# QuentinFuxa/WhisperLiveKit

Hardware: AMD Instinct MI355X
Metric: audio seconds transcribed per second (1/RTF), Whisper-base EN simul_whisper AlignAtt, 0.5 s chunks (higher is better)
Workload: dtype f32; 1 GPU; base.en simul_whisper, 1 stream(s) over 1 GPU(s) (1 per GPU), 30 s 16 kHz speech-like stream, 0.5 s chunks, beam 1, frame_threshold 25, seeded random weights, synthetic vocabulary; model=base.en, streams_total=1

## Files before the change

### include/wlk_hip.h

```cpp
#ifndef WLK_HIP_H
#define WLK_HIP_H

#include <stdint.h>

#ifdef __cplusplus
extern "C" {
#endif

#define WLK_OK 0
#define WLK_ERR_ARG (-1)
#define WLK_ERR_HIP (-2)
#define WLK_ERR_STATE (-3)
#define WLK_ERR_CAPACITY (-4)

typedef struct wlk_model wlk_model;
typedef struct wlk_session wlk_session;

typedef struct wlk_dims {
    int32_t n_mels, n_audio_ctx, n_audio_state, n_audio_head, n_audio_layer;
    int32_t n_vocab, n_text_ctx, n_text_state, n_text_head, n_text_layer;
} wlk_dims;

const char* wlk_last_error(void);
int wlk_abi_version(void);
int wlk_device_count(void);

int wlk_arena_floats(const wlk_dims* dims, uint64_t* n_floats);
int wlk_tensor_lookup(const wlk_dims* dims, const char* packed_name, uint64_t* offset_floats,
                      uint64_t* numel);
int wlk_tensor_name(const wlk_dims* dims, int index, const char** name);

int wlk_model_create(const wlk_dims* dims, int device, float* arena_dev, wlk_model** out);
int wlk_model_arena(wlk_model* m, float** arena_dev, uint64_t* n_floats);
int wlk_model_upload(wlk_model* m, const char* packed_name, const float* host, uint64_t numel);
int wlk_model_set_alignment_heads(wlk_model* m, const int32_t* layer_head_pairs, int n_pairs);
int wlk_model_finalize(wlk_model* m);
int wlk_model_destroy(wlk_model* m);

int wlk_session_create(wlk_model* m, int beam, int max_audio_samples, wlk_session** out);
int wlk_session_destroy(wlk_session* s);
// ... 180 lines not shown
int wlk_diag_linear_time(int m, int n, int k, int flags, int force_gemv, int reps, float* us_per_launch);
int wlk_diag_linear_ln(const float* a, const float* w, const float* bias, const float* gamma, const float* beta,
                       int m, int n, int k, int force_gemv, float* c);
int wlk_diag_layernorm(const float* x, const float* gamma, const float* beta, int rows, int d, float* y);
int wlk_diag_prefill_stack(wlk_session** sessions, const int64_t* tokens, const int32_t* n_tok, const int32_t* sot_index, int32_t n,
                           int32_t* taken);
int wlk_engine_prefill_stats(wlk_model* m, uint64_t* batches, uint64_t* sessions);
int wlk_diag_encoder_attention_time(int t, int d, int n_head, int k_splits, int reps, float* us_per_launch);
int wlk_diag_encoder_attention(const float* qkv, int t, int d, int n_head, float* out);
int wlk_diag_wave_ops(const float* in64, float* out640, float* ref640);
int wlk_diag_linear_x3(const float* a, const float* w, const float* bias, int m, int n, int k, int flags, float scale,
                       int scale_cols, float* c);
int wlk_diag_linear_x3_time(int m, int n, int k, int flags, int reps, float* us_per_launch);
int wlk_diag_layernorm_x3(const float* x, const float* gamma, const float* beta, int rows, int d, float* y);
int wlk_diag_encoder_attention_x3(const float* qkv, int t, int d, int n_head, float* out);
int wlk_diag_encoder_attention_x3_time(int t, int d, int n_head, int reps, float* us_per_launch);
int wlk_diag_qkv_x3_attention(const float* x, const float* w, const float* bias, int t, int d, int n_head, float scale,
                              float* out_epilogue, float* out_packed);

#ifdef __cplusplus
}
#endif
#endif
```

### whisperlivekit_amd/_lib.py

```python
from __future__ import annotations

import ctypes as C
import os
import threading
from typing import Optional


_LIB_NAME = "libwlk_hip.so"
_lock = threading.Lock()
_lib: Optional[C.CDLL] = None


class WlkError(RuntimeError):
    """Raised for every non-zero status of the C ABI (message from wlk_last_error())."""


class Dims(C.Structure):
    _fields_ = [(n, C.c_int32) for n in (
        "n_mels", "n_audio_ctx", "n_audio_state", "n_audio_head", "n_audio_layer",
        "n_vocab", "n_text_ctx", "n_text_state", "n_text_head", "n_text_layer")]


class SfDims(C.Structure):
    _fields_ = [(n, C.c_int32) for n in (
# ... 45 lines not shown
    os.environ["GPU_MAX_HW_QUEUES"] = str(int(n))
    return True


def lib_path() -> str:
    return os.environ.get("WLK_HIP_LIB", os.path.join(os.path.dirname(os.path.abspath(__file__)), _LIB_NAME))


def _declare(lib: C.CDLL) -> None:
    p, i32, u64, f32p, i32p = C.c_void_p, C.c_int32, C.c_uint64, C.POINTER(C.c_float), C.POINTER(C.c_int32)
    cint = C.c_int
    sig = {
        "wlk_last_error": (C.c_char_p, []),
        "wlk_abi_version": (cint, []),
        "wlk_device_count": (cint, []),
        "wlk_arena_floats": (cint, [C.POINTER(Dims), C.POINTER(u64)]),
        "wlk_tensor_lookup": (cint, [C.POINTER(Dims), C.c_char_p, C.POINTER(u64), C.POINTER(u64)]),
        "wlk_tensor_name": (cint, [C.POINTER(Dims), cint, C.POINTER(C.c_char_p)]),
        "wlk_model_create": (cint, [C.POINTER(Dims), cint, p, C.POINTER(p)]),
        "wlk_model_arena": (cint, [p, C.POINTER(p), C.POINTER(u64)]),
        "wlk_model_upload": (cint, [p, C.c_char_p, p, u64]),
        "wlk_model_set_alignment_heads": (cint, [p, p, cint]),
        "wlk_model_finalize": (cint, [p]),
        "wlk_model_destroy": (cint, [p]),
        "wlk_session_create": (cint, [p, cint, cint, C.POINTER(p)]),
        "wlk_session_destroy": (cint, [p]),
        "wlk_session_set_debug": (cint, [p, cint]),
        "wlk_audio_append": (cint, [p, p, cint]),
        "wlk_audio_append_pcm16": (cint, [p, p, cint]),
        "wlk_audio_append_zeros": (cint, [p, cint]),
# ... 75 lines not shown
        "wlk_log_mel": (cint, [C.c_void_p, C.POINTER(C.c_float), C.c_int64, C.c_int32, C.POINTER(C.c_float), C.c_uint64,
                               C.POINTER(C.c_int32)]),
        "wlk_find_alignment": (cint, [C.c_void_p, C.POINTER(C.c_int64), C.c_int32, C.c_int32, C.c_int32, C.c_int32, C.c_float,
                                      C.POINTER(C.c_float), C.POINTER(C.c_int8), C.POINTER(C.c_float)]),
        "wlk_diag_linear_time": (cint, [cint, cint, cint, cint, cint, cint, C.POINTER(C.c_float)]),
        "wlk_diag_linear_ln": (cint, [p, p, p, p, p, cint, cint, cint, cint, p]),
        "wlk_diag_layernorm": (cint, [p, p, p, cint, cint, p]),
        "wlk_diag_encoder_attention_time": (cint, [cint, cint, cint, cint, cint, C.POINTER(C.c_float)]),
        "wlk_diag_encoder_attention": (cint, [p, cint, cint, cint, p]),
        "wlk_diag_wave_ops": (cint, [p, p, p]),
        "wlk_diag_env_refresh": (cint, []),
        "wlk_diag_linear_x3": (cint, [p, p, p, cint, cint, cint, cint, C.c_float, cint, p]),
        "wlk_diag_linear_x3_time": (cint, [cint, cint, cint, cint, cint, C.POINTER(C.c_float)]),
        "wlk_diag_layernorm_x3": (cint, [p, p, p, cint, cint, p]),
        "wlk_diag_encoder_attention_x3": (cint, [p, cint, cint, cint, p]),
        "wlk_diag_encoder_attention_x3_time": (cint, [cint, cint, cint, cint, C.POINTER(C.c_float)]),
        "wlk_diag_qkv_x3_attention": (cint, [p, p, p, cint, cint, cint, C.c_float, p, p]),
    }
    for name, (res, args) in sig.items():
        try:
            fn = getattr(lib, name)
        except AttributeError:
            if "WLK_HIP_LIB" in os.environ and name.startswith("wlk_diag_"):
                continue
            raise
        fn.restype = res
        fn.argtypes = args


EXPORTED_SYMBOLS = (
    "wlk_last_error", "wlk_abi_version", "wlk_device_count", "wlk_arena_floats", "wlk_tensor_lookup",
    "wlk_tensor_name", "wlk_model_create", "wlk_model_arena", "wlk_model_upload",
    "wlk_model_set_alignment_heads", "wlk_model_finalize", "wlk_model_destroy", "wlk_session_create",
    "wlk_session_destroy", "wlk_session_set_debug", "wlk_audio_append", "wlk_audio_append_pcm16", "wlk_audio_append_zeros",
    "wlk_audio_drop_front", "wlk_audio_clear", "wlk_audio_len", "wlk_encode", "wlk_decode",
    "wlk_no_speech_prob", "wlk_rules_set", "wlk_pick_greedy", "wlk_select", "wlk_kv_reorder", "wlk_sync", "wlk_decode_until_stop", "wlk_engine_attach", "wlk_engine_detach",
    "wlk_engine_stats", "wlk_engine_encode_stats", "wlk_engine_prefill_stats", "wlk_diag_prefill_stack", "wlk_job_create",
    "wlk_job_begin_step", "wlk_job_no_speech", "wlk_job_adjustments", "wlk_job_consume", "wlk_job_result",
    "wlk_job_destroy", "wlk_export", "wlk_session_step_stats", "wlk_prof_begin",
    "wlk_prof_end", "wlk_melspec_create", "wlk_melspec_run", "wlk_melspec_destroy",
    "wlk_sf_arena_floats", "wlk_sf_tensor_lookup", "wlk_sf_tensor_name", "wlk_sf_create", "wlk_sf_upload",
    "wlk_sf_finalize", "wlk_sf_step", "wlk_sf_step_pcm", "wlk_sf_stats", "wlk_sf_export", "wlk_sf_destroy",
    "wlk_vad_weights_floats", "wlk_vad_tensor_lookup", "wlk_vad_tensor_name", "wlk_vad_create", "wlk_vad_destroy",
    "wlk_vad_stream_create", "wlk_vad_stream_reset", "wlk_vad_stream_run", "wlk_vad_stream_state",
    "wlk_vad_stream_destroy",
    "wlk_dtw", "wlk_encode_mel", "wlk_log_mel", "wlk_find_alignment",
    "wlk_nllb_arena_floats", "wlk_nllb_tensor_lookup", "wlk_nllb_tensor_name", "wlk_nllb_create", "wlk_nllb_upload",
    "wlk_nllb_finalize", "wlk_nllb_destroy", "wlk_nllb_session_create", "wlk_nllb_session_destroy", "wlk_nllb_encode",
    "wlk_nllb_decode", "wlk_nllb_step", "wlk_nllb_kv_reorder", "wlk_nllb_topk", "wlk_nllb_export", "wlk_nllb_sync",
    "wlk_diag_last_error", "wlk_diag_linear", "wlk_diag_linear_time", "wlk_diag_linear_ln", "wlk_diag_layernorm",
    "wlk_diag_encoder_attention", "wlk_diag_encoder_attention_time", "wlk_diag_wave_ops", "wlk_diag_env_refresh",
    "wlk_diag_linear_x3", "wlk_diag_linear_x3_time", "wlk_diag_layernorm_x3",
    "wlk_diag_encoder_attention_x3", "wlk_diag_encoder_attention_x3_time", "wlk_diag_qkv_x3_attention",
)


def load() -> C.CDLL:
    global _lib
    if _lib is not None:
        return _lib
    with _lock:
        if _lib is None:
            path = lib_path()
            if not os.path.exists(path):
                raise WlkError(
                    f"{path} not found: build it with `python -m whisperlivekit_amd.build` "
                    "(hipcc, gfx950). There is no CPU fallback for the HIP backend.")
            try:
# ... 21 lines not shown
```

### whisperlivekit_amd/csrc/api.hip

```cpp
#include <cmath>
#include <cstdio>
#include <cstdlib>
#include <atomic>
#include <chrono>
#include <cstring>
#include <map>
#include <memory>
#include <mutex>
#include <string>
#include <vector>

#include "../../include/wlk_hip.h"
#include "common.h"
#include "internal.h"

namespace wlk {

namespace {
struct UtilStream {
    std::mutex mu;
    hipStream_t stream = nullptr;
};
UtilStream g_util[64];
UtilStream& util_of_current_device() {
// ... 112 lines not shown
    L.fc1w = m->w(p + "fc1.w"); L.fc1b = m->w(p + "fc1.b");
    L.fc2w = m->w(p + "fc2.w"); L.fc2b = m->w(p + "fc2.b");
    if (cross) {
        L.lnxw = m->w(p + "lnx.w"); L.lnxb = m->w(p + "lnx.b");
        L.xqw = m->w(p + "xq.w"); L.xqb = m->w(p + "xq.b");
        L.xkvw = m->w(p + "xkv.w"); L.xkvb = m->w(p + "xkv.b");
        L.xoutw = m->w(p + "xout.w"); L.xoutb = m->w(p + "xout.b");
    }
    return L;
}

extern "C" {

const char* wlk_last_error(void) { return g_last_error.c_str(); }
int wlk_abi_version(void) { return 2; }

int wlk_device_count(void) {
    int n = 0;
    if (hipGetDeviceCount(&n) != hipSuccess) {
        (void)hipGetLastError();
        return 0;
    }
    return n;
}

int wlk_arena_floats(const wlk_dims* dims, uint64_t* n_floats) {
    if (int rc = check_dims(dims)) return rc;
    if (!n_floats) return fail(WLK_ERR_ARG, "n_floats is NULL");
    build_layout(*dims, n_floats);
    return WLK_OK;
// ... 1727 lines not shown
```

### whisperlivekit_amd/csrc/attention_x3.hip

```cpp
#include <atomic>
#include <cstdlib>
#include <type_traits>

#include "common.h"
#include "wave_ops.h"
#include "x3.h"

namespace wlk {

namespace {
typedef float af32x4 __attribute__((ext_vector_type(4)));

constexpr int AX_QT = 64, AX_KT = 32;
constexpr int AX_K_ROW = 384;
constexpr int AX_V_ROW = 192;
constexpr int AX_K_BYTES = AX_KT * AX_K_ROW;
constexpr int AX_V_BYTES = 64 * AX_V_ROW;
constexpr int AX_TILE_BYTES = AX_K_BYTES + AX_V_BYTES;
constexpr int AX_SLOT_BYTES = 2 * AX_TILE_BYTES;
constexpr int AX_NB = 3, AX_DT = AX_NB - 1;
constexpr int AX_NPW = AX_SLOT_BYTES / 1024 / 8;
constexpr size_t AX_LDS_BYTES = (size_t)AX_NB * AX_SLOT_BYTES;
constexpr int AX_PA[6] = {2, 0, 1, 1, 0, 0}, AX_PB[6] = {0, 2, 1, 0, 1, 0};

template <int N, int I = 0, typename F>
__device__ __forceinline__ void ax_static_for(F&& f) {
    if constexpr (I < N) {
        f(std::integral_constant<int, I>{});
        ax_static_for<N, I + 1>(f);
    }
}
__device__ __forceinline__ void ax_read12(af32x4 (&f)[12], const unsigned (&addr)[12], unsigned off) {
#pragma unroll
    for (int t = 0; t < 12; ++t) asm volatile("ds_read_b128 %0, %1" : "=v"(f[t]) : "v"(addr[t] + off));
}
__device__ __forceinline__ void ax_wait12(af32x4 (&f)[12]) {
    asm volatile("s_waitcnt lgkmcnt(0)" : "+v"(f[0]), "+v"(f[1]), "+v"(f[2]), "+v"(f[3]), "+v"(f[4]), "+v"(f[5]));
    asm volatile("" : "+v"(f[6]), "+v"(f[7]), "+v"(f[8]), "+v"(f[9]), "+v"(f[10]), "+v"(f[11]));
}
__device__ __forceinline__ void ax_split8(const float (&v)[8], bf16x8 (&out)[3]) {
#pragma unroll
    for (int e = 0; e < 8; ++e) {
        const X3Triple t = x3_split(v[e]);
        out[0][e] = t.h;
        out[1][e] = t.m;
        out[2][e] = t.l;
    }
}
__host__ __device__ inline int ax_vt_key(int u, int e) { return 4 * u + (e & 3) + 16 * (e >> 2); }
// ... 81 lines not shown
                const int key = min((2 * sc + stream_of[i]) * AX_KT + key_row[i], T - 1);
                p = src[i] + (long)key * row_qk;
            } else {
                p = src[i] + (long)min(sc, (n_tiles - 1 - stream_of[i]) / 2) * adv[i];
            }
            __builtin_amdgcn_global_load_lds((const __attribute__((address_space(1))) void*)p,
                                             (__attribute__((address_space(3))) void*)(lds + slot * AX_SLOT_BYTES + (wave + 8 * i) * 1024),
                                             16, 0, 0);
        });
    };
    issue_step(0);
    issue_step(1);

    const unsigned lds_base = (unsigned)(size_t)(__attribute__((address_space(3))) unsigned char*)lds;
    const unsigned tile_base = lds_base + (unsigned)ks * AX_TILE_BYTES;
    unsigned k_addr[12], v_addr[12];
#pragma unroll
    for (int kb = 0; kb < 2; ++kb)
#pragma unroll
        for (int kstep = 0; kstep < 2; ++kstep)
#pragma unroll
            for (int p = 0; p < 3; ++p) {
                const int row = 16 * kb + c;
                k_addr[kb * 6 + kstep * 3 + p] = tile_base + (unsigned)(row * AX_K_ROW) + (unsigned)((((4 * kstep + g) ^ (row & 7)) * 3 + p) * 16);
            }
#pragma unroll
    for (int db = 0; db < 4; ++db)
#pragma unroll
        for (int p = 0; p < 3; ++p) {
            const int row = 16 * db + c;
            v_addr[db * 3 + p] = tile_base + AX_K_BYTES + (unsigned)(row * AX_V_ROW) + (unsigned)(((g ^ ((row >> 1) & 3)) * 3 + p) * 16);
        }
    af32x4 o[4];
#pragma unroll
    for (int db = 0; db < 4; ++db) o[db] = af32x4{0.f, 0.f, 0.f, 0.f};
    float m_run = -INFINITY, l_run = 0.f;

    af32x4 vf[12];
    float s[8];
    auto phase_s = [&](int tile, unsigned off) {
        af32x4 kf[12];
        ax_read12(kf, k_addr, off);
        ax_read12(vf, v_addr, off);
        ax_wait12(kf);
        af32x4 s2[2] = {af32x4{0.f, 0.f, 0.f, 0.f}, af32x4{0.f, 0.f, 0.f, 0.f}};
        ax_static_for<24>([&](auto X) {
            constexpr int x = decltype(X)::value;
            constexpr int t = x / 4, kstep = (x / 2) % 2, kb = x % 2;
            s2[kb] = __builtin_amdgcn_mfma_f32_16x16x32_bf16(__builtin_bit_cast(bf16x8, kf[kb * 6 + kstep * 3 + AX_PA[t]]),
                                                             qf[kstep * 3 + AX_PB[t]], s2[kb], 0, 0, 0);
        });
#pragma unroll
        for (int i = 0; i < 4; ++i) { s[i] = s2[0][i]; s[4 + i] = s2[1][i]; }
        const int key0 = tile * AX_KT;
        if (__builtin_amdgcn_readfirstlane(key0 + AX_KT > T)) {
#pragma unroll
            for (int i = 0; i < 8; ++i)
                if (key0 + 16 * (i >> 2) + 4 * g + (i & 3) >= T) s[i] = -INFINITY;
// ... 87 lines not shown
#pragma unroll
        for (int i = 0; i < 8; ++i) {
            const int q = qg * 8 + i;
            const int qrow = q0 + q;
            const int w0 = q >> 4, w1 = w0 + 4;
            const float m0 = Ms[w0 * 16 + (q & 15)], m1 = Ms[w1 * 16 + (q & 15)];
            const float M = fmaxf(m0, m1);
            const float e0 = m0 == -INFINITY ? 0.f : expf(m0 - M), e1 = m1 == -INFINITY ? 0.f : expf(m1 - M);
            const float L = e0 * Ls[w0 * 16 + (q & 15)] + e1 * Ls[w1 * 16 + (q & 15)];
            const float acc = e0 * Os[(w0 * 16 + (q & 15)) * O_LD + dd] + e1 * Os[(w1 * 16 + (q & 15)) * O_LD + dd];
            if (qrow < T) aout[(long)qrow * a.ldo + head * 64 + dd] = acc / L;
        }
    }
}

__global__ __launch_bounds__(256) void x3_pack_qkv_kernel(const float* __restrict__ qkv, unsigned short* __restrict__ out, int T, int d,
                                                          long vt_off, long vt_ld) {
    const long n_qk = (long)T * (2 * d / 8), n_vt = (long)d * (vt_ld / 8);
    const long idx = (long)blockIdx.x * 256 + threadIdx.x;
    float v[8];
    if (idx < n_qk) {
        const int row = (int)(idx / (2 * d / 8)), c = (int)(idx - (long)row * (2 * d / 8));
#pragma unroll
        for (int e = 0; e < 8; ++e) v[e] = qkv[(long)row * 3 * d + 8 * c + e];
        x3_store_chunk(out + (long)row * 3 * (2 * d) + (long)c * 24, v);
    } else if (idx < n_qk + n_vt) {
        const long j = idx - n_qk;
        const int dcol = (int)(j / (vt_ld / 8)), u = (int)(j - (long)dcol * (vt_ld / 8));
#pragma unroll
        for (int e = 0; e < 8; ++e) {
// ... 7 lines not shown
void launch_x3_pack_qkv(const LaunchCtx& ctx, const float* qkv, unsigned short* out, int T, int d, long vt_off, long vt_ld) {
    const long n = (long)T * (2 * d / 8) + (long)d * (vt_ld / 8);
    KernelScope ks(ctx, "x3_pack_qkv");
    hipLaunchKernelGGL(x3_pack_qkv_kernel, dim3((unsigned)((n + 255) / 256)), dim3(256), 0, ctx.stream, qkv, out, T, d, vt_off, vt_ld);
    WLK_HIP(hipGetLastError());
}

bool enc_attention_x3_enabled() {
    static const bool on = [] {
        const char* e = getenv("WLK_X3_ATTN");
        return !(e && e[0] == '0');
    }();
    return on;
}

void launch_encoder_attention_x3(const LaunchCtx& ctx, const unsigned short* qk3, long ldqk, long vt_off, long vt_ld, float* out,
                                 long ldo, int T, int d, int n_head, const PtrTable* z, int batch, bool x3_out) {
    if (d != n_head * 64 || ldqk % 8 != 0 || vt_ld % 32 != 0 || vt_ld < ((T + 31) / 32) * 32 || T < 64)
        throw std::invalid_argument("x3 attention: unsupported shape");
    static std::atomic<uint64_t> configured{0};
    int dev = 0;
    WLK_HIP(hipGetDevice(&dev));
    if (!(configured.load(std::memory_order_acquire) >> (dev & 63) & 1)) {
        WLK_HIP(hipFuncSetAttribute(reinterpret_cast<const void*>(&enc_attention_x3_kernel<0>), hipFuncAttributeMaxDynamicSharedMemorySize, (int)AX_LDS_BYTES));
        WLK_HIP(hipFuncSetAttribute(reinterpret_cast<const void*>(&enc_attention_x3_kernel<1>), hipFuncAttributeMaxDynamicSharedMemorySize, (int)AX_LDS_BYTES));
        WLK_HIP(hipFuncSetAttribute(reinterpret_cast<const void*>(&enc_attention_x3_kernel<2>), hipFuncAttributeMaxDynamicSharedMemorySize, (int)AX_LDS_BYTES));
        WLK_HIP(hipFuncSetAttribute(reinterpret_cast<const void*>(&enc_attention_x3_kernel<3>), hipFuncAttributeMaxDynamicSharedMemorySize, (int)AX_LDS_BYTES));
        configured.fetch_or(1ull << (dev & 63), std::memory_order_release);
    }
    AttnX3Args a{};
    a.qk3 = qk3; a.ldqk = ldqk; a.vt_off = vt_off; a.vt_ld = vt_ld; a.out = out; a.ldo = ldo; a.T = T; a.d = d; a.n_head = n_head;
    a.batch = batch;
    a.x3_out = x3_out ? 1 : 0;
    if (x3_out && ldo % 8 != 0) throw std::invalid_argument("x3 attention: X3 result rows need ldo % 8 == 0");
    if (batch > 0) a.z = *z;
    const int q_tiles = (T + AX_QT - 1) / AX_QT;
    KernelScope ks(ctx, "enc_attention_x3", (batch > 0 ? batch : 1) * 4.0 * (double)T * T * 64 * n_head, 0.0);
    static const int abl = [] {
        const char* e = getenv("WLK_X3_ATTN_ABL");
        return e ? atoi(e) : 0;
    }();
    const dim3 grid(q_tiles * n_head, batch > 0 ? batch : 1);
    if (abl == 1) hipLaunchKernelGGL(enc_attention_x3_kernel<1>, grid, dim3(512), AX_LDS_BYTES, ctx.stream, a);
    else if (abl == 2) hipLaunchKernelGGL(enc_attention_x3_kernel<2>, grid, dim3(512), AX_LDS_BYTES, ctx.stream, a);
    else if (abl == 3) hipLaunchKernelGGL(enc_attention_x3_kernel<3>, grid, dim3(512), AX_LDS_BYTES, ctx.stream, a);
    else hipLaunchKernelGGL(enc_attention_x3_kernel<0>, grid, dim3(512), AX_LDS_BYTES, ctx.stream, a);
    WLK_HIP(hipGetLastError());
}

}
```

### whisperlivekit_amd/csrc/common.h

```cpp
#pragma once
#include <hip/hip_runtime.h>

#include <cstdint>
#include <stdexcept>
#include <mutex>
#include <string>

namespace wlk {

constexpr int kNFft = 400;
constexpr int kHop = 160;
constexpr int kNFreq = 201;
constexpr int kMelFrames = 3000;
constexpr int kPadSamples = 480000;
constexpr int kHeadDim = 64;
constexpr int kAlignWindow = 16;

struct HipError : std::runtime_error {
    using std::runtime_error::runtime_error;
};

inline void hip_check(hipError_t e, const char* what, const char* file, int line) {
    if (e != hipSuccess) {
        throw HipError(std::string(what) + " failed: " + hipGetErrorString(e) + " (" + file + ":" +
// ... 204 lines not shown
    long vt_ld = 0;
    bool x3_out = false;
    PtrTable z;
};
bool gemm_x3_wide_applicable(int M, int N, int K, long lda);
void launch_gemm_x3(const LaunchCtx& ctx, const X3GemmArgs& g, const char* tag);
size_t x3_w_elems(int n, int k);
void launch_x3_pack_w(const LaunchCtx& ctx, const float* src, long ld_src, unsigned short* dst, int n, int k);
void launch_x3_pack(const LaunchCtx& ctx, const float* src, long ld_src, unsigned short* dst, long ld_dst, int rows, int cols);
void launch_x3_unpack(const LaunchCtx& ctx, const unsigned short* src, long ld_src, float* dst, long ld_dst, int rows, int cols);

inline long x3_attn_vt_ld(int T) { return ((long)T + 31) / 32 * 32; }
inline long x3_attn_vt_off(int T, int d) { return (long)T * 3 * 2 * d; }
inline size_t x3_attn_image_elems(int T, int d) { return (size_t)x3_attn_vt_off(T, d) + (size_t)d * 3 * x3_attn_vt_ld(T); }
bool enc_attention_x3_enabled();
void launch_encoder_attention_x3(const LaunchCtx& ctx, const unsigned short* qk3, long ldqk, long vt_off, long vt_ld, float* out,
                                 long ldo, int T, int d, int n_head, const PtrTable* z, int batch, bool x3_out = false);
void launch_x3_pack_qkv(const LaunchCtx& ctx, const float* qkv, unsigned short* out, int T, int d, long vt_off, long vt_ld);

void launch_layernorm(const LaunchCtx& ctx, const float* x, long ldx, const float* gamma, const float* beta,
                      float* y, long ldy, int rows, int d, const char* tag);
void launch_layernorm_batched(const LaunchCtx& ctx, const PtrTable& z, int batch, long ldx, const float* gamma,
                              const float* beta, long ldy, int rows, int d, const char* tag);
void launch_layernorm_x3(const LaunchCtx& ctx, const float* x, long ldx, const float* gamma, const float* beta,
                         unsigned short* y3, long ldy3, int rows, int d, const char* tag);
void launch_layernorm_x3_batched(const LaunchCtx& ctx, const PtrTable& z, int batch, long ldx, const float* gamma,
                                 const float* beta, long ldy3, int rows, int d, const char* tag);

struct MelArgs {
    const float* audio;
// ... 199 lines not shown
```

### whisperlivekit_amd/csrc/diag.hip

```cpp
#include <cstdio>
#include <cstdlib>
#include <vector>

#include "../../include/wlk_hip.h"
#include "common.h"
#include "internal.h"
#include "wave_ops.h"

using namespace wlk;

namespace {
thread_local std::string g_diag_error;
struct DevBuf {
    float* p = nullptr;
    explicit DevBuf(size_t n, const float* host = nullptr) {
        WLK_HIP(hipMalloc(reinterpret_cast<void**>(&p), std::max<size_t>(n, 1) * sizeof(float)));
        if (host) WLK_HIP(hipMemcpy(p, host, n * sizeof(float), hipMemcpyHostToDevice));
    }
    ~DevBuf() { (void)hipFree(p); }
};
template <typename F>
int run(F&& f) {
    try {
        f();
// ... 366 lines not shown
int wlk_diag_encoder_attention_x3(const float* qkv, int t, int d, int n_head, float* out) {
    return run([&]() {
        DevBuf Q((size_t)t * 3 * d, qkv), O((size_t)t * d);
        unsigned short* img = nullptr;
        const size_t n = x3_attn_image_elems(t, d);
        WLK_HIP(hipMalloc(reinterpret_cast<void**>(&img), n * sizeof(unsigned short)));
        LaunchCtx ctx;
        launch_x3_pack_qkv(ctx, Q.p, img, t, d, x3_attn_vt_off(t, d), x3_attn_vt_ld(t));
        launch_encoder_attention_x3(ctx, img, 2L * d, x3_attn_vt_off(t, d), x3_attn_vt_ld(t), O.p, d, t, d, n_head, nullptr, 0);
        WLK_HIP(hipDeviceSynchronize());
        WLK_HIP(hipMemcpy(out, O.p, (size_t)t * d * sizeof(float), hipMemcpyDeviceToHost));
        (void)hipFree(img);
    });
}

int wlk_diag_qkv_x3_attention(const float* x, const float* w, const float* bias, int t, int d, int n_head, float scale,
                              float* out_epilogue, float* out_packed) {
    return run([&]() {
        DevBuf X((size_t)t * d, x), W((size_t)3 * d * d, w), B((size_t)3 * d, bias), QKV((size_t)t * 3 * d), O((size_t)t * d);
        unsigned short *x3 = nullptr, *w3 = nullptr, *img = nullptr;
        const size_t n_img = x3_attn_image_elems(t, d);
        WLK_HIP(hipMalloc(reinterpret_cast<void**>(&x3), (size_t)t * 3 * d * sizeof(unsigned short)));
        WLK_HIP(hipMalloc(reinterpret_cast<void**>(&w3), x3_w_elems(3 * d, d) * sizeof(unsigned short)));
        WLK_HIP(hipMalloc(reinterpret_cast<void**>(&img), n_img * sizeof(unsigned short)));
        LaunchCtx ctx;
        launch_x3_pack(ctx, X.p, d, x3, d, t, d);
        launch_x3_pack_w(ctx, W.p, d, w3, 3 * d, d);
        X3GemmArgs g;
        g.A3 = x3; g.lda = d; g.W3 = w3; g.bias = B.p; g.M = t; g.N = 3 * d; g.K = d;
        g.flags = kGemmScaleCols; g.scale = scale; g.scale_cols = 2 * d;
// ... 55 lines not shown
```

### whisperlivekit_amd/csrc/gemm_f32.hip

```cpp
#include <algorithm>
#include <atomic>
#include <cstdio>
#include <cstdlib>
#include <type_traits>

#include "common.h"
#include "wave_ops.h"
#include "align_body.h"

namespace wlk {

typedef float f32x16 __attribute__((ext_vector_type(16)));
typedef float f32x4 __attribute__((ext_vector_type(4)));
typedef unsigned int u32x4 __attribute__((ext_vector_type(4)));

constexpr int BK = 32, LDS_LD = BK + 4;

__device__ __forceinline__ float gelu_erf(float x) {
    return 0.5f * x * (1.0f + erff(x * 0.70710678118654752440f));
}

template <int NA, int NW>
struct Stage {
    float4 a[NA], w[NW];
// ... 1005 lines not shown

static bool kwave16_enabled() {
    static const bool on = [] {
        const char* e = getenv("WLK_KWAVE16");
        return !(e && e[0] == '0');
    }();
    return on;
}

static bool gemm_can_fuse_layernorm(int M, int N, int K) {
    return kwave16_enabled() && M > 8 && M <= 128 && gemm_takes_kwave(M, N, K) && ksplit_tile(M, N, K).tm == 0 &&
           (K == 384 || K == 512 || K == 768 || K == 1024 || K == 1280);
}
static std::atomic<int> g_prefill_ln_fuse{-1};
void x3_refresh_env_switches();
void refresh_env_switches() {
    g_prefill_ln_fuse.store(-1, std::memory_order_relaxed);
    x3_refresh_env_switches();
}
bool gemm_fuses_layernorm(int M, int N, int K) {
    int on = g_prefill_ln_fuse.load(std::memory_order_relaxed);
    if (on < 0) {
        const char* e = getenv("WLK_PREFILL_LN_FUSE");
        on = e && e[0] == '1';
        g_prefill_ln_fuse.store(on, std::memory_order_relaxed);
    }
    return on && gemm_can_fuse_layernorm(M, N, K);
}

void launch_gemm(const LaunchCtx& ctx, const GemmArgs& g, const char* tag) {
    if (g.M <= 0 || g.N <= 0) return;
    if (g.K % 4 != 0 || g.lda % 4 != 0) throw std::invalid_argument("gemm: K and lda must be multiples of 4");
    if ((((long)g.M - 1) * g.lda + g.K) * 4 >= (1L << 31) || (long)g.N * g.K * 4 >= (1L << 31))
// ... 728 lines not shown
```

Measured before the change: 200.8 audio_s/s.

## Add 48-query 12-wave X3 encoder attention kernel and use ds_read immediate offsets

Adds an alternative encoder attention kernel that tiles 48 query rows over 12 waves. It splits keys four ways within a workgroup, double-buffers V, and merges the partial softmax results in LDS. The kernel is selectable via an environment variable or a CU-count heuristic, to improve workgroup-to-CU balance. The existing kernel now encodes LDS read offsets as instruction immediates instead of keeping 24 precomputed address registers, which reduces VGPR pressure. Diagnostics for batched attention and the query-row heuristic are added.

```diff
diff --git a/include/wlk_hip.h b/include/wlk_hip.h
--- a/include/wlk_hip.h
+++ b/include/wlk_hip.h
@@ -24,6 +24,7 @@
 const char* wlk_last_error(void);
 int wlk_abi_version(void);
 int wlk_device_count(void);
+int wlk_diag_x3_attn_query_rows(int t, int n_head, int n_cu);
 
 int wlk_arena_floats(const wlk_dims* dims, uint64_t* n_floats);
 int wlk_tensor_lookup(const wlk_dims* dims, const char* packed_name, uint64_t* offset_floats,
@@ -234,6 +235,7 @@
 int wlk_diag_linear_x3_time(int m, int n, int k, int flags, int reps, float* us_per_launch);
 int wlk_diag_layernorm_x3(const float* x, const float* gamma, const float* beta, int rows, int d, float* y);
 int wlk_diag_encoder_attention_x3(const float* qkv, int t, int d, int n_head, float* out);
+int wlk_diag_encoder_attention_x3_batch(const float* qkv, int batch, int t, int d, int n_head, int x3_out, int batched, void* out);
 int wlk_diag_encoder_attention_x3_time(int t, int d, int n_head, int reps, float* us_per_launch);
 int wlk_diag_qkv_x3_attention(const float* x, const float* w, const float* bias, int t, int d, int n_head, float scale,
                               float* out_epilogue, float* out_packed);
diff --git a/whisperlivekit_amd/_lib.py b/whisperlivekit_amd/_lib.py
--- a/whisperlivekit_amd/_lib.py
+++ b/whisperlivekit_amd/_lib.py
@@ -83,6 +83,7 @@
         "wlk_last_error": (C.c_char_p, []),
         "wlk_abi_version": (cint, []),
         "wlk_device_count": (cint, []),
+        "wlk_diag_x3_attn_query_rows": (cint, [cint, cint, cint]),
         "wlk_arena_floats": (cint, [C.POINTER(Dims), C.POINTER(u64)]),
         "wlk_tensor_lookup": (cint, [C.POINTER(Dims), C.c_char_p, C.POINTER(u64), C.POINTER(u64)]),
         "wlk_tensor_name": (cint, [C.POINTER(Dims), cint, C.POINTER(C.c_char_p)]),
@@ -188,6 +189,7 @@
         "wlk_diag_linear_x3_time": (cint, [cint, cint, cint, cint, cint, C.POINTER(C.c_float)]),
         "wlk_diag_layernorm_x3": (cint, [p, p, p, cint, cint, p]),
         "wlk_diag_encoder_attention_x3": (cint, [p, cint, cint, cint, p]),
+        "wlk_diag_encoder_attention_x3_batch": (cint, [p, cint, cint, cint, cint, cint, cint, p]),
         "wlk_diag_encoder_attention_x3_time": (cint, [cint, cint, cint, cint, C.POINTER(C.c_float)]),
         "wlk_diag_qkv_x3_attention": (cint, [p, p, p, cint, cint, cint, C.c_float, p, p]),
     }
@@ -203,7 +205,7 @@
 
 
 EXPORTED_SYMBOLS = (
-    "wlk_last_error", "wlk_abi_version", "wlk_device_count", "wlk_arena_floats", "wlk_tensor_lookup",
+    "wlk_last_error", "wlk_abi_version", "wlk_device_count", "wlk_diag_x3_attn_query_rows", "wlk_arena_floats", "wlk_tensor_lookup",
     "wlk_tensor_name", "wlk_model_create", "wlk_model_arena", "wlk_model_upload",
     "wlk_model_set_alignment_heads", "wlk_model_finalize", "wlk_model_destroy", "wlk_session_create",
     "wlk_session_destroy", "wlk_session_set_debug", "wlk_audio_append", "wlk_audio_append_pcm16", "wlk_audio_append_zeros",
@@ -225,7 +227,7 @@
     "wlk_diag_last_error", "wlk_diag_linear", "wlk_diag_linear_time", "wlk_diag_linear_ln", "wlk_diag_layernorm",
     "wlk_diag_encoder_attention", "wlk_diag_encoder_attention_time", "wlk_diag_wave_ops", "wlk_diag_env_refresh",
     "wlk_diag_linear_x3", "wlk_diag_linear_x3_time", "wlk_diag_layernorm_x3",
-    "wlk_diag_encoder_attention_x3", "wlk_diag_encoder_attention_x3_time", "wlk_diag_qkv_x3_attention",
+    "wlk_diag_encoder_attention_x3", "wlk_diag_encoder_attention_x3_batch", "wlk_diag_encoder_attention_x3_time", "wlk_diag_qkv_x3_attention",
 )
 
 
diff --git a/whisperlivekit_amd/csrc/api.hip b/whisperlivekit_amd/csrc/api.hip
--- a/whisperlivekit_amd/csrc/api.hip
+++ b/whisperlivekit_amd/csrc/api.hip
@@ -150,6 +150,8 @@
 
 const char* wlk_last_error(void) { return g_last_error.c_str(); }
 int wlk_abi_version(void) { return 2; }
+
+int wlk_diag_x3_attn_query_rows(int T, int n_head, int n_cu) { return wlk::x3_attn_query_rows(T, n_head, n_cu); }
 
 int wlk_device_count(void) {
     int n = 0;
diff --git a/whisperlivekit_amd/csrc/attention_x3.hip b/whisperlivekit_amd/csrc/attention_x3.hip
--- a/whisperlivekit_amd/csrc/attention_x3.hip
+++ b/whisperlivekit_amd/csrc/attention_x3.hip
@@ -30,9 +30,10 @@
         ax_static_for<N, I + 1>(f);
     }
 }
-__device__ __forceinline__ void ax_read12(af32x4 (&f)[12], const unsigned (&addr)[12], unsigned off) {
-#pragma unroll
-    for (int t = 0; t < 12; ++t) asm volatile("ds_read_b128 %0, %1" : "=v"(f[t]) : "v"(addr[t] + off));
+template <int OFF>
+__device__ __forceinline__ void ax_read(af32x4& f, unsigned addr) {
+    static_assert(OFF >= 0 && OFF < 65536, "ds_read offset field");
+    asm volatile("ds_read_b128 %0, %1 offset:%2" : "=v"(f) : "v"(addr), "i"(OFF));
 }
 __device__ __forceinline__ void ax_wait12(af32x4 (&f)[12]) {
     asm volatile("s_waitcnt lgkmcnt(0)" : "+v"(f[0]), "+v"(f[1]), "+v"(f[2]), "+v"(f[3]), "+v"(f[4]), "+v"(f[5]));
@@ -144,23 +145,9 @@
 
     const unsigned lds_base = (unsigned)(size_t)(__attribute__((address_space(3))) unsigned char*)lds;
     const unsigned tile_base = lds_base + (unsigned)ks * AX_TILE_BYTES;
-    unsigned k_addr[12], v_addr[12];
-#pragma unroll
-    for (int kb = 0; kb < 2; ++kb)
-#pragma unroll
-        for (int kstep = 0; kstep < 2; ++kstep)
-#pragma unroll
-            for (int p = 0; p < 3; ++p) {
-                const int row = 16 * kb + c;
-                k_addr[kb * 6 + kstep * 3 + p] = tile_base + (unsigned)(row * AX_K_ROW) + (unsigned)((((4 * kstep + g) ^ (row & 7)) * 3 + p) * 16);
-            }
-#pragma unroll
-    for (int db = 0; db < 4; ++db)
-#pragma unroll
-        for (int p = 0; p < 3; ++p) {
-            const int row = 16 * db + c;
-            v_addr[db * 3 + p] = tile_base + AX_K_BYTES + (unsigned)(row * AX_V_ROW) + (unsigned)(((g ^ ((row >> 1) & 3)) * 3 + p) * 16);
-        }
+    const unsigned k_a0 = tile_base + (unsigned)(c * AX_K_ROW + (g ^ (c & 7)) * 3 * 16);
+    const unsigned k_a1 = tile_base + (unsigned)(c * AX_K_ROW + ((4 + g) ^ (c & 7)) * 3 * 16);
+    const unsigned v_a = tile_base + (unsigned)(AX_K_BYTES + c * AX_V_ROW + (g ^ ((c >> 1) & 3)) * 3 * 16);
     af32x4 o[4];
 #pragma unroll
     for (int db = 0; db < 4; ++db) o[db] = af32x4{0.f, 0.f, 0.f, 0.f};
@@ -170,8 +157,16 @@
     float s[8];
     auto phase_s = [&](int tile, unsigned off) {
         af32x4 kf[12];
-        ax_read12(kf, k_addr, off);
-        ax_read12(vf, v_addr, off);
+        const unsigned ka0 = k_a0 + off, ka1 = k_a1 + off, va = v_a + off;
+        ax_static_for<12>([&](auto X) {
+            constexpr int x = decltype(X)::value;
+            constexpr int kb = x / 6, kstep = (x / 3) % 2, p = x % 3;
+            ax_read<kb * 16 * AX_K_ROW + p * 16>(kf[x], kstep ? ka1 : ka0);
+        });
+        ax_static_for<12>([&](auto X) {
+            constexpr int x = decltype(X)::value;
+            ax_read<(x / 3) * 16 * AX_V_ROW + (x % 3) * 16>(vf[x], va);
+        });
         ax_wait12(kf);
         af32x4 s2[2] = {af32x4{0.f, 0.f, 0.f, 0.f}, af32x4{0.f, 0.f, 0.f, 0.f}};
         ax_static_for<24>([&](auto X) {
@@ -289,6 +284,234 @@
     }
 }
 
+constexpr int A4_QT = 48, A4_NS = 4, A4_WAVES = 12;
+constexpr int A4_K_REGION = A4_NS * AX_K_BYTES;
+constexpr int A4_V_REGION = A4_NS * AX_V_BYTES;
+constexpr size_t A4_LDS_BYTES = (size_t)A4_K_REGION + 2 * (size_t)A4_V_REGION;
+constexpr int A4_O_LD = 68;
+static_assert(A4_LDS_BYTES <= 160 * 1024, "48-query X3 attention: LDS budget");
+static_assert((A4_WAVES * 16 * A4_O_LD + 2 * A4_WAVES * 16) * 4 <= (int)A4_LDS_BYTES, "48-query X3 attention: epilogue image");
+static_assert(AX_K_BYTES == A4_WAVES * 1024 && AX_V_BYTES == A4_WAVES * 1024, "one 1 KiB DMA piece per wave and tile");
+
+template <int ABL>
+__global__ __launch_bounds__(768) void enc_attention_x3_q48_kernel(AttnX3Args a) {
+    asm volatile("" ::"s"(a.qk3), "s"(a.ldqk), "s"(a.vt_off), "s"(a.vt_ld), "s"(a.out), "s"(a.ldo), "s"(a.T), "s"(a.d), "s"(a.n_head),
+                 "s"(a.batch));
+    __builtin_amdgcn_sched_barrier(0);
+    extern __shared__ __attribute__((aligned(1024))) unsigned char lds[];
+    const int lane = threadIdx.x & 63;
+    const int wave = __builtin_amdgcn_readfirstlane(threadIdx.x >> 6);
+    const bool batched = a.batch > 0;
+    const unsigned short* const qk3 = batched ? reinterpret_cast<const unsigned short*>(table_at(a.z.in, blockIdx.y)) : a.qk3;
+    float* const aout = batched ? table_at(a.z.out, blockIdx.y) : a.out;
+    const int T = a.T;
+    const int head = blockIdx.x % a.n_head;
+    const int q0 = (blockIdx.x / a.n_head) * A4_QT;
+    const int n_tiles = (T + AX_KT - 1) / AX_KT;
+    const int n_steps = (n_tiles + A4_NS - 1) / A4_NS;
+    const long row_qk = 3 * a.ldqk * 2, row_vt = 3 * a.vt_ld * 2;
+    const int qs = wave % 3, ks = wave / 3;
+    const int c = lane & 15, g = lane >> 4;
+
+    bf16x8 qf[6];
+    {
+        const int q = min(q0 + 16 * qs + c, T - 1);
+        const char* qp = reinterpret_cast<const char*>(qk3) + (long)q * row_qk + (long)(head * 8) * 48;
+#pragma unroll
+        for (int kstep = 0; kstep < 2; ++kstep)
+#pragma unroll
+            for (int p = 0; p < 3; ++p)
+                qf[kstep * 3 + p] = __builtin_bit_cast(bf16x8, *reinterpret_cast<const x3_u32x4*>(qp + ((4 * kstep + g) * 3 + p) * 16));
+    }
+    const int in_tile = 1024 * wave + 16 * lane;
+    const int k_row = in_tile / AX_K_ROW;
+    const char* k_src;
+    const char* v_src;
+    {
+        const int up = (in_tile - k_row * AX_K_ROW) >> 4;
+        const int unit = ((up / 3) ^ (k_row & 7)) * 3 + up % 3;
+        k_src = reinterpret_cast<const char*>(qk3) + (long)(a.d / 8 + head * 8) * 48 + unit * 16;
+        const int row = in_tile / AX_V_ROW;
+        const int vup = (in_tile - row * AX_V_ROW) >> 4;
+        const int vunit = ((vup / 3) ^ ((row >> 1) & 3)) * 3 + vup % 3;
+        v_src = reinterpret_cast<const char*>(qk3 + a.vt_off) + (long)(head * 64 + row) * row_vt + vunit * 16;
+    }
+    const char* const k_src_row = k_src + (long)k_row * row_qk;
+    auto issue_step = [&](int step) {
+        if constexpr (ABL >= 2) return;
+        const int vbuf = step & 1;
+        const bool whole = (A4_NS * step + A4_NS) * AX_KT <= T;
+        ax_static_for<A4_NS>([&](auto I) {
+            constexpr int i = decltype(I)::value;
+            const int tile = A4_NS * step + i;
+            const int key0 = tile * AX_KT;
+            const char* pk;
+            if (whole) pk = k_src_row + (long)key0 * row_qk;
+            else pk = k_src + (long)min(key0 + k_row, T - 1) * row_qk;
+            const char* pv = v_src + (long)min(tile, n_tiles - 1) * ((AX_KT / 8) * 48);
+            __builtin_amdgcn_global_load_lds((const __attribute__((address_space(1))) void*)pk,
+                                             (__attribute__((address_space(3))) void*)(lds + i * AX_K_BYTES + wave * 1024), 16, 0, 0);
+            __builtin_amdgcn_global_load_lds((const __attribute__((address_space(1))) void*)pv,
+                                             (__attribute__((address_space(3))) void*)(lds + A4_K_REGION + vbuf * A4_V_REGION + i * AX_V_BYTES + wave * 1024),
+                                             16, 0, 0);
+        });
+    };
+    issue_step(0);
+
+    const unsigned lds_base = (unsigned)(size_t)(__attribute__((address_space(3))) unsigned char*)lds;
+    const unsigned k_row_base = lds_base + (unsigned)(ks * AX_K_BYTES + c * AX_K_ROW);
+    const unsigned k_a0 = k_row_base + (unsigned)((g ^ (c & 7)) * 3 * 16);
+    const unsigned k_a1 = k_row_base + (unsigned)(((4 + g) ^ (c & 7)) * 3 * 16);
+    const unsigned v_a = lds_base + (unsigned)(A4_K_REGION + ks * AX_V_BYTES + c * AX_V_ROW + (g ^ ((c >> 1) & 3)) * 3 * 16);
+
+    af32x4 o[4];
+#pragma unroll
+    for (int db = 0; db < 4; ++db) o[db] = af32x4{0.f, 0.f, 0.f, 0.f};
+    float m_run = -INFINITY, l_run = 0.f;
+
+    for (int st = 0; st < n_steps; ++st) {
+        asm volatile("s_waitcnt vmcnt(0)" ::: "memory");
+        __builtin_amdgcn_s_barrier();
+        const int tile = A4_NS * st + ks;
+        const bool active = ABL != 1 && tile < n_tiles;
+        float s[8];
+        if (active) {
+            af32x4 kf[12];
+            ax_static_for<12>([&](auto X) {
+                constexpr int x = decltype(X)::value;
+                constexpr int kb = x / 6, kstep = (x / 3) % 2, p = x % 3;
+                ax_read<kb * 16 * AX_K_ROW + p * 16>(kf[x], kstep ? k_a1 : k_a0);
+            });
+            ax_wait12(kf);
+            af32x4 s2[2] = {af32x4{0.f, 0.f, 0.f, 0.f}, af32x4{0.f, 0.f, 0.f, 0.f}};
+            ax_static_for<24>([&](auto X) {
+                constexpr int x = decltype(X)::value;
+                constexpr int t = x / 4, kstep = (x / 2) % 2, kb = x % 2;
+                s2[kb] = __builtin_amdgcn_mfma_f32_16x16x32_bf16(__builtin_bit_cast(bf16x8, kf[kb * 6 + kstep * 3 + AX_PA[t]]),
+                                                                 qf[kstep * 3 + AX_PB[t]], s2[kb], 0, 0, 0);
+            });
+#pragma unroll
+            for (int i = 0; i < 4; ++i) { s[i] = s2[0][i]; s[4 + i] = s2[1][i]; }
+            const int key0 = tile * AX_KT;
+            if (__builtin_amdgcn_readfirstlane(key0 + AX_KT > T)) {
+#pragma unroll
+                for (int i = 0; i < 8; ++i)
+                    if (key0 + 16 * (i >> 2) + 4 * g + (i & 3) >= T) s[i] = -INFINITY;
+            }
+        }
+        __builtin_amdgcn_s_barrier();
+        if (st + 1 < n_steps) issue_step(st + 1);
+        if (active) {
+            af32x4 vf[12];
+            const unsigned va = v_a + (unsigned)((st & 1) * A4_V_REGION);
+            ax_static_for<12>([&](auto X) {
+                constexpr int x = decltype(X)::value;
+                ax_read<(x / 3) * 16 * AX_V_ROW + (x % 3) * 16>(vf[x], va);
+            });
+            bf16x8 pf[3];
+            if constexpr (ABL != 3) {
+                float mt = fmaxf(fmaxf(fmaxf(s[0], s[1]), fmaxf(s[2], s[3])), fmaxf(fmaxf(s[4], s[5]), fmaxf(s[6], s[7])));
+                mt = fmaxf(mt, wave_xor<16>(mt));
+                mt = fmaxf(mt, wave_xor<32>(mt));
+                const float m_new = fmaxf(m_run, mt);
+                const float alpha = __expf(m_run - m_new);
+                float rs = 0.f;
+#pragma unroll
+                for (int i = 0; i < 8; ++i) {
+                    s[i] = __expf(s[i] - m_new);
+                    rs += s[i];
+                }
+                rs += wave_xor<16>(rs);
+                rs += wave_xor<32>(rs);
+                l_run = l_run * alpha + rs;
+                m_run = m_new;
+                if (__builtin_amdgcn_ballot_w64(alpha != 1.0f) != 0) {
+#pragma unroll
+                    for (int db = 0; db < 4; ++db) o[db] *= alpha;
+                }
+                ax_split8(s, pf);
+                ax_wait12(vf);
+            } else {
+                ax_wait12(vf);
+#pragma unroll
+                for (int p = 0; p < 3; ++p) pf[p] = __builtin_bit_cast(bf16x8, vf[p]);
+            }
+            ax_static_for<24>([&](auto X) {
+                constexpr int x = decltype(X)::value;
+                constexpr int t = x / 4, db = x % 4;
+                o[db] = __builtin_amdgcn_mfma_f32_16x16x32_bf16(__builtin_bit_cast(bf16x8, vf[db * 3 + AX_PA[t]]), pf[AX_PB[t]], o[db], 0, 0, 0);
+            });
+        }
+    }
+    asm volatile("s_waitcnt vmcnt(0) lgkmcnt(0)" ::: "memory");
+    __builtin_amdgcn_s_barrier();
+
+    float* Os = reinterpret_cast<float*>(lds);
+    float* Ms = Os + A4_WAVES * 16 * A4_O_LD;
+    float* Ls = Ms + A4_WAVES * 16;
+#pragma unroll
+    for (int db = 0; db < 4; ++db)
+#pragma unroll
+        for (int i = 0; i < 4; ++i) Os[(wave * 16 + c) * A4_O_LD + 16 * db + 4 * g + i] = o[db][i];
+    if (g == 0) {
+        Ms[wave * 16 + c] = m_run;
+        Ls[wave * 16 + c] = l_run;
+    }
+    asm volatile("s_waitcnt lgkmcnt(0)" ::: "memory");
+    __builtin_amdgcn_s_barrier();
+    auto weights = [&](int q, int (&row)[4], float (&e)[4]) -> float {
+        float m[4];
+#pragma unroll
+        for (int k = 0; k < A4_NS; ++k) {
+            row[k] = ((q >> 4) + 3 * k) * 16 + (q & 15);
+            m[k] = Ms[row[k]];
+        }
+        const float M = fmaxf(fmaxf(m[0], m[1]), fmaxf(m[2], m[3]));
+        float L = 0.f;
+#pragma unroll
+        for (int k = 0; k < A4_NS; ++k) {
+            e[k] = m[k] == -INFINITY ? 0.f : expf(m[k] - M);
+            L = L + e[k] * Ls[row[k]];
+        }
+        return L;
+    };
+    const int tid = threadIdx.x;
+    if (a.x3_out) {
+        if (tid < A4_QT * 8) {
+            const int q = tid >> 3, ch = tid & 7;
+            const int qrow = q0 + q;
+            int row[4];
+            float e[4];
+            const float L = weights(q, row, e);
+            float v[8];
+#pragma unroll
+            for (int j = 0; j < 8; ++j) {
+                const int dd = 8 * ch + j;
+                float acc = 0.f;
+#pragma unroll
+                for (int k = 0; k < A4_NS; ++k) acc = acc + e[k] * Os[row[k] * A4_O_LD + dd];
+                v[j] = acc / L;
+            }
+            if (qrow < T)
+                x3_store_chunk(reinterpret_cast<unsigned short*>(aout) + (long)qrow * 3 * a.ldo + (long)(head * 8 + ch) * 24, v);
+        }
+    } else {
+        const int dd = tid & 63, qg = tid >> 6;
+#pragma unroll
+        for (int i = 0; i < A4_QT / A4_WAVES; ++i) {
+            const int q = qg * (A4_QT / A4_WAVES) + i;
+            const int qrow = q0 + q;
+            int row[4];
+            float e[4];
+            const float L = weights(q, row, e);
+            float acc = 0.f;
+#pragma unroll
+            for (int k = 0; k < A4_NS; ++k) acc = acc + e[k] * Os[row[k] * A4_O_LD + dd];
+            if (qrow < T) aout[(long)qrow * a.ldo + head * 64 + dd] = acc / L;
+        }
+    }
+}
+
 __global__ __launch_bounds__(256) void x3_pack_qkv_kernel(const float* __restrict__ qkv, unsigned short* __restrict__ out, int T, int d,
                                                           long vt_off, long vt_ld) {
     const long n_qk = (long)T * (2 * d / 8), n_vt = (long)d * (vt_ld / 8);
@@ -326,11 +549,32 @@
     return on;
 }
 
+int x3_attn_query_rows(int T, int n_head, int n_cu) {
+    const long cu = n_cu > 0 ? n_cu : 1;
+    const long wg64 = (T + AX_QT - 1) / AX_QT * (long)n_head, wg48 = (T + A4_QT - 1) / A4_QT * (long)n_head;
+    const long r64 = (wg64 + cu - 1) / cu, r48 = (wg48 + cu - 1) / cu;
+    return 3 * r48 < 4 * r64 ? A4_QT : AX_QT;
+}
+
+static std::atomic<int> g_x3_attn_qt{-1};
+void x3_attn_refresh_env_switches() { g_x3_attn_qt.store(-1, std::memory_order_relaxed); }
+
+static int x3_attn_qt_mode() {
+    int m = g_x3_attn_qt.load(std::memory_order_relaxed);
+    if (m < 0) {
+        const char* e = getenv("WLK_X3_ATTN_QT");
+        m = !e ? 0 : atoi(e) == A4_QT ? 1 : (e[0] == 'a' || e[0] == 'A') ? 2 : 0;
+        g_x3_attn_qt.store(m, std::memory_order_relaxed);
+    }
+    return m;
+}
+
 void launch_encoder_attention_x3(const LaunchCtx& ctx, const unsigned short* qk3, long ldqk, long vt_off, long vt_ld, float* out,
                                  long ldo, int T, int d, int n_head, const PtrTable* z, int batch, bool x3_out) {
     if (d != n_head * 64 || ldqk % 8 != 0 || vt_ld % 32 != 0 || vt_ld < ((T + 31) / 32) * 32 || T < 64)
         throw std::invalid_argument("x3 attention: unsupported shape");
     static std::atomic<uint64_t> configured{0};
+    static std::atomic<int> cu_count[64];
     int dev = 0;
     WLK_HIP(hipGetDevice(&dev));
     if (!(configured.load(std::memory_order_acquire) >> (dev & 63) & 1)) {
@@ -338,6 +582,13 @@
         WLK_HIP(hipFuncSetAttribute(reinterpret_cast<const void*>(&enc_attention_x3_kernel<1>), hipFuncAttributeMaxDynamicSharedMemorySize, (int)AX_LDS_BYTES));
         WLK_HIP(hipFuncSetAttribute(reinterpret_cast<const void*>(&enc_attention_x3_kernel<2>), hipFuncAttributeMaxDynamicSharedMemorySize, (int)AX_LDS_BYTES));
         WLK_HIP(hipFuncSetAttribute(reinterpret_cast<const void*>(&enc_attention_x3_kernel<3>), hipFuncAttributeMaxDynamicSharedMemorySize, (int)AX_LDS_BYTES));
+        WLK_HIP(hipFuncSetAttribute(reinterpret_cast<const void*>(&enc_attention_x3_q48_kernel<0>), hipFuncAttributeMaxDynamicSharedMemorySize, (int)A4_LDS_BYTES));
+        WLK_HIP(hipFuncSetAttribute(reinterpret_cast<const void*>(&enc_attention_x3_q48_kernel<1>), hipFuncAttributeMaxDynamicSharedMemorySize, (int)A4_LDS_BYTES));
+        WLK_HIP(hipFuncSetAttribute(reinterpret_cast<const void*>(&enc_attention_x3_q48_kernel<2>), hipFuncAttributeMaxDynamicSharedMemorySize, (int)A4_LDS_BYTES));
+        WLK_HIP(hipFuncSetAttribute(reinterpret_cast<const void*>(&enc_attention_x3_q48_kernel<3>), hipFuncAttributeMaxDynamicSharedMemorySize, (int)A4_LDS_BYTES));
+        int cus = 0;
+        WLK_HIP(hipDeviceGetAttribute(&cus, hipDeviceAttributeMultiprocessorCount, dev));
+        cu_count[dev & 63].store(cus, std::memory_order_relaxed);
         configured.fetch_or(1ull << (dev & 63), std::memory_order_release);
     }
     AttnX3Args a{};
@@ -346,17 +597,27 @@
     a.x3_out = x3_out ? 1 : 0;
     if (x3_out && ldo % 8 != 0) throw std::invalid_argument("x3 attention: X3 result rows need ldo % 8 == 0");
     if (batch > 0) a.z = *z;
-    const int q_tiles = (T + AX_QT - 1) / AX_QT;
+    const int mode = x3_attn_qt_mode();
+    const int qt = mode == 0 ? AX_QT : mode == 1 ? A4_QT : x3_attn_query_rows(T, n_head, cu_count[dev & 63].load(std::memory_order_relaxed));
+    const int q_tiles = (T + qt - 1) / qt;
     KernelScope ks(ctx, "enc_attention_x3", (batch > 0 ? batch : 1) * 4.0 * (double)T * T * 64 * n_head, 0.0);
     static const int abl = [] {
         const char* e = getenv("WLK_X3_ATTN_ABL");
         return e ? atoi(e) : 0;
     }();
     const dim3 grid(q_tiles * n_head, batch > 0 ? batch : 1);
-    if (abl == 1) hipLaunchKernelGGL(enc_attention_x3_kernel<1>, grid, dim3(512), AX_LDS_BYTES, ctx.stream, a);
-    else if (abl == 2) hipLaunchKernelGGL(enc_attention_x3_kernel<2>, grid, dim3(512), AX_LDS_BYTES, ctx.stream, a);
-    else if (abl == 3) hipLaunchKernelGGL(enc_attention_x3_kernel<3>, grid, dim3(512), AX_LDS_BYTES, ctx.stream, a);
-    else hipLaunchKernelGGL(enc_attention_x3_kernel<0>, grid, dim3(512), AX_LDS_BYTES, ctx.stream, a);
+    if (qt == A4_QT) {
+        const dim3 block(64 * A4_WAVES);
+        if (abl == 1) hipLaunchKernelGGL(enc_attention_x3_q48_kernel<1>, grid, block, A4_LDS_BYTES, ctx.stream, a);
+        else if (abl == 2) hipLaunchKernelGGL(enc_attention_x3_q48_kernel<2>, grid, block, A4_LDS_BYTES, ctx.stream, a);
+        else if (abl == 3) hipLaunchKernelGGL(enc_attention_x3_q48_kernel<3>, grid, block, A4_LDS_BYTES, ctx.stream, a);
+        else hipLaunchKernelGGL(enc_attention_x3_q48_kernel<0>, grid, block, A4_LDS_BYTES, ctx.stream, a);
+    } else {
+        if (abl == 1) hipLaunchKernelGGL(enc_attention_x3_kernel<1>, grid, dim3(512), AX_LDS_BYTES, ctx.stream, a);
+        else if (abl == 2) hipLaunchKernelGGL(enc_attention_x3_kernel<2>, grid, dim3(512), AX_LDS_BYTES, ctx.stream, a);
+        else if (abl == 3) hipLaunchKernelGGL(enc_attention_x3_kernel<3>, grid, dim3(512), AX_LDS_BYTES, ctx.stream, a);
+        else hipLaunchKernelGGL(enc_attention_x3_kernel<0>, grid, dim3(512), AX_LDS_BYTES, ctx.stream, a);
+    }
     WLK_HIP(hipGetLastError());
 }
 
diff --git a/whisperlivekit_amd/csrc/common.h b/whisperlivekit_amd/csrc/common.h
--- a/whisperlivekit_amd/csrc/common.h
+++ b/whisperlivekit_amd/csrc/common.h
@@ -242,6 +242,7 @@
 inline long x3_attn_vt_off(int T, int d) { return (long)T * 3 * 2 * d; }
 inline size_t x3_attn_image_elems(int T, int d) { return (size_t)x3_attn_vt_off(T, d) + (size_t)d * 3 * x3_attn_vt_ld(T); }
 bool enc_attention_x3_enabled();
+int x3_attn_query_rows(int T, int n_head, int n_cu);
 void launch_encoder_attention_x3(const LaunchCtx& ctx, const unsigned short* qk3, long ldqk, long vt_off, long vt_ld, float* out,
                                  long ldo, int T, int d, int n_head, const PtrTable* z, int batch, bool x3_out = false);
 void launch_x3_pack_qkv(const LaunchCtx& ctx, const float* qkv, unsigned short* out, int T, int d, long vt_off, long vt_ld);
diff --git a/whisperlivekit_amd/csrc/diag.hip b/whisperlivekit_amd/csrc/diag.hip
--- a/whisperlivekit_amd/csrc/diag.hip
+++ b/whisperlivekit_amd/csrc/diag.hip
@@ -404,6 +404,34 @@
     });
 }
 
+int wlk_diag_encoder_attention_x3_batch(const float* qkv, int batch, int t, int d, int n_head, int x3_out, int batched, void* out) {
+    return run([&]() {
+        if (batch < 1 || batch > kMaxBatch) throw std::invalid_argument("batch out of range");
+        const size_t n = x3_attn_image_elems(t, d), res_bytes = (size_t)t * d * (x3_out ? 6 : 4);
+        DevBuf Q((size_t)batch * t * 3 * d, qkv), O((size_t)batch * res_bytes / 4);
+        unsigned short* img = nullptr;
+        WLK_HIP(hipMalloc(reinterpret_cast<void**>(&img), (size_t)batch * n * sizeof(unsigned short)));
+        LaunchCtx ctx;
+        PtrTable z{};
+        for (int i = 0; i < batch; ++i) {
+            launch_x3_pack_qkv(ctx, Q.p + (size_t)i * t * 3 * d, img + (size_t)i * n, t, d, x3_attn_vt_off(t, d), x3_attn_vt_ld(t));
+            z.in[i] = reinterpret_cast<const float*>(img + (size_t)i * n);
+            z.out[i] = reinterpret_cast<float*>(reinterpret_cast<char*>(O.p) + (size_t)i * res_bytes);
+        }
+        if (batched) {
+            launch_encoder_attention_x3(ctx, nullptr, 2L * d, x3_attn_vt_off(t, d), x3_attn_vt_ld(t), nullptr, d, t, d, n_head, &z, batch,
+                                        x3_out != 0);
+        } else {
+            for (int i = 0; i < batch; ++i)
+                launch_encoder_attention_x3(ctx, img + (size_t)i * n, 2L * d, x3_attn_vt_off(t, d), x3_attn_vt_ld(t), z.out[i], d, t, d,
+                                            n_head, nullptr, 0, x3_out != 0);
+        }
+        WLK_HIP(hipDeviceSynchronize());
+        WLK_HIP(hipMemcpy(out, O.p, (size_t)batch * res_bytes, hipMemcpyDeviceToHost));
+        (void)hipFree(img);
+    });
+}
+
 int wlk_diag_qkv_x3_attention(const float* x, const float* w, const float* bias, int t, int d, int n_head, float scale,
                               float* out_epilogue, float* out_packed) {
     return run([&]() {
diff --git a/whisperlivekit_amd/csrc/gemm_f32.hip b/whisperlivekit_amd/csrc/gemm_f32.hip
--- a/whisperlivekit_amd/csrc/gemm_f32.hip
+++ b/whisperlivekit_amd/csrc/gemm_f32.hip
@@ -1043,9 +1043,11 @@
 }
 static std::atomic<int> g_prefill_ln_fuse{-1};
 void x3_refresh_env_switches();
+void x3_attn_refresh_env_switches();
 void refresh_env_switches() {
     g_prefill_ln_fuse.store(-1, std::memory_order_relaxed);
     x3_refresh_env_switches();
+    x3_attn_refresh_env_switches();
 }
 bool gemm_fuses_layernorm(int M, int N, int K) {
     int on = g_prefill_ln_fuse.load(std::memory_order_relaxed);
```

Result: no change. 199.8 audio_s/s (median of 6 runs) (-0.5%).
